# LIS-TU-Berlin/SVN-ICP

Measured on AMD Instinct MI355X. Metric: scan-pair registrations/sec at N particles x M source pts, 1/2/4/8 GPU, higher is better.
Workload: dtype f64; 1 GPU; C3: 128 particles SVN-ICP, 131072-pt source vs 262144-pt target, K=100, I=20, max_dist=1.0, lr=1.0, SVNFullGrad=False, correspondence=fast, early stop off; synthetic 64-beam scans (seed 20250718); particles=128, target_points=262144, knn_count=100, parallelism=single GPU

## Files before the change

### svn-icp_amd/csrc/api.hip

```cpp
#include "../../include/svnicp_hip.h"

#include <cmath>
#include <algorithm>
#include <cstdio>
#include <cstdlib>
#include <cstring>
#include <string>
#include <vector>

#include "device_buffer.hpp"
#include "kernels.hpp"
#include "stage_a_host.hpp"
#include "stage_b_host.hpp"

using namespace svnicp;
using namespace svnicp_host;

namespace {

struct CloudState {
  DevBuf<double> src, tgt;
  bool src_set = false, tgt_set = false;
};

// ... 313 lines not shown
  c->st.init_in_flight = true;
  c->st.host_stats_valid = false;
  const bool first = !c->run.particles_set || P != c->P;
  if (first && c->shard.row_world > 1) { c->shard.row_world = 1; c->shard.row_rank = 0; c->shard.B_total = 0; }
  c->P = P;
  if (!c->shard.set || first) { c->shard.p_lo = 0; c->shard.p_hi = P; c->shard.set = false; }
  HIPCHK(c, launch_init_particles(c->st.init_pose.p, P, c->pose0, c->prm.mode, c->st.R.p, c->st.t.p, c->st.Rtot.p, c->st.pose_out.p,
                                  (first || c->prm.mode == SVNICP_MODE_SVN) ? 1 : 0, c->st.eul.p, c->stream));
  c->run.particles_set = true;
  return SVNICP_OK;
}

int svnicp_set_initial_mean(svnicp_ctx* c, const double R0[9], const double t0[3]) {
  CTX_CHECK(c);
  if (!R0 || !t0) return fail(c, SVNICP_ERR_INVALID, "svnicp_set_initial_mean: null argument");
  std::memcpy(c->pose0.R0, R0, 9 * sizeof(double));
  std::memcpy(c->pose0.t0, t0, 3 * sizeof(double));
  c->run.have_candidates = false;
  return SVNICP_OK;
}

int svnicp_set_k(svnicp_ctx* c, int k) {
  CTX_CHECK(c);
  if (k < 1) return fail(c, SVNICP_ERR_INVALID, "svnicp_set_k: k >= 1 required");
  c->K = k;
  c->run.have_candidates = false;
  return SVNICP_OK;
}

int svnicp_set_max_dist(svnicp_ctx* c, double md) {
  CTX_CHECK(c);
  c->prm.max_dist = md;
  return SVNICP_OK;
}

int svnicp_set_option(svnicp_ctx* c, const char* name, const char* value) {
  CTX_CHECK(c);
  if (!name || !value) return fail(c, SVNICP_ERR_INVALID, "svnicp_set_option: null argument");
  const std::string k(name), v(value);
  Tuning& t = c->tune;
  auto num = [&](int lo, int hi, int* out) { char* end = nullptr; const long x = strtol(v.c_str(), &end, 10);
                                             if (end == v.c_str() || *end || x < lo || x > hi) return false; *out = (int)x; return true; };
  bool ok = true;
  if (k == "knn") { if (v == "auto") t.knn = {}; else if (v == "v1") t.knn = {false, KnnKernel::Stream}; else if (v == "v2") t.knn = {false, KnnKernel::SeededScan};
                    else if (v == "brute") t.knn = {false, KnnKernel::Brute}; else if (v == "tiles") t.knn = {false, KnnKernel::Tiles}; else ok = false; }
  else if (k == "fallback_sliced_max") ok = num(-1, 1 << 20, &t.fallback_sliced_max);
  else if (k == "accum") { if (v == "f64") t.accum = 0; else if (v == "valu") t.accum = 1; else if (v == "split") t.accum = 3; else ok = false; }
  else if (k == "update") { if (v == "auto") t.update_fused = 0; else if (v == "fused") t.update_fused = 1; else ok = false; }
  else if (k == "fused_update_max_p") ok = num(1, 700, &t.fused_update_max_p);
  else if (k == "wgpcu") { int x = 0, y = 0; ok = sscanf(v.c_str(), "%d,%d", &x, &y) == 2 && x >= 0 && x <= 64 && y >= 0 && y <= 16; if (ok) { t.wgpcu_search = x; t.wgpcu_accum = y; } }
  else if (k == "tp") ok = num(0, 1 << 16, &t.tp);
  else if (k == "debug") ok = num(0, 1, &t.debug);
  else if (k == "scan_split") ok = num(0, 16, &t.scan_split);
  else if (k == "group_stride") ok = num(0, 1 << 30, &t.group_stride);
  else if (k == "accum_min_steps") ok = num(0, 1 << 20, &t.accum_min_steps);
  else if (k == "brute_qb") { ok = num(0, 6, &t.brute_qb); }
  else if (k == "single") { if (v == "fused") t.single_fused = 1; else if (v == "split") t.single_fused = 0; else ok = false; }
  else if (k == "chain") { if (v == "auto") { t.small_chain = 1; t.persistent = 0; } else if (v == "persistent") { t.small_chain = 1; t.persistent = 1; }
                           else if (v == "general") { t.small_chain = 0; t.persistent = 0; } else ok = false; }
  else if (k == "median") { if (v == "auto") t.median_inline = -1; else if (v == "stream") t.median_inline = 0; else if (v == "inline") t.median_inline = 1; else ok = false; }
  else if (k == "correspondence") { if (v == "fast") t.full_corr = 0; else if (v == "full") t.full_corr = 1; else ok = false; }
  else return fail(c, SVNICP_ERR_INVALID, "svnicp_set_option: unknown option '" + k + "'");
  if (!ok) return fail(c, SVNICP_ERR_INVALID, "svnicp_set_option: bad value '" + v + "' for option '" + k + "'");
  c->run.have_candidates = false;
  c->sa.held = TargetLayout::None;
  if (c->run.began) c->st.step = plan_step(registration_facts(c, c->pl.on), c->tune, c->sb.plan);
  return SVNICP_OK;
}

int svnicp_set_shard(svnicp_ctx* c, int p_lo, int p_hi) {
  CTX_CHECK(c);
  if (!c->run.particles_set || p_lo < 0 || p_hi > c->P || p_lo > p_hi)
    return fail(c, SVNICP_ERR_INVALID, "svnicp_set_shard: need 0 <= p_lo <= p_hi <= P after svnicp_set_particles");
  c->shard.p_lo = p_lo; c->shard.p_hi = p_hi; c->shard.set = true;
  return SVNICP_OK;
}

int svnicp_set_row_shard(svnicp_ctx* c, int row_rank, int row_world, int64_t total_source_points) {
  CTX_CHECK(c);
  if (!c->run.particles_set || row_world < 1 || row_rank < 0 || row_rank >= row_world || (row_world > 1 && total_source_points < 1))
    return fail(c, SVNICP_ERR_INVALID, "svnicp_set_row_shard: need 0 <= row_rank < row_world and the whole scan's point count, after svnicp_set_particles");
  if (bind(c)) return SVNICP_ERR_HIP;
  c->shard.row_rank = row_rank; c->shard.row_world = row_world;
  c->shard.B_total = row_world > 1 ? total_source_points : 0;
  if (row_world > 1) {
    HIPCHK(c, c->shard.rank_sums.ensure((size_t)row_world * c->P * kNSums));
    HIPCHK(c, hipMemsetAsync(c->shard.rank_sums.p, 0, (size_t)row_world * c->P * kNSums * sizeof(double), c->stream));
  }
  return SVNICP_OK;
}

void* svnicp_rank_sums_devptr(svnicp_ctx* c) { return (c && c->shard.row_world > 1) ? (void*)c->shard.rank_sums.p : nullptr; }

static bool normal_pass_due(const svnicp_ctx* c) {
  return c->pl.on && !c->pl.supplied && !(c->pl.estimated && c->pl.est_k == c->pl.normal_k);
}

static int prepare_plane(svnicp_ctx* c);
int svnicp_align_begin(svnicp_ctx* c) {
  CTX_CHECK(c);
  if (!c->cloud.src_set || !c->cloud.tgt_set || !c->run.particles_set)
    return fail(c, SVNICP_ERR_INVALID, "svnicp_align: svnicp_set_clouds and svnicp_set_particles must come first");
  if (bind(c)) return SVNICP_ERR_HIP;
  const int I = c->prm.iterations, P = c->P;
  const int64_t B = c->B;
  const bool plane = c->pl.residual == SVNICP_RESIDUAL_PLANE;
// ... 774 lines not shown
```

### svn-icp_amd/csrc/kernels.hpp

```cpp
#pragma once
#include "device_math.hpp"
#include "registration_plan.hpp"
#include "stage_a_plan.hpp"

namespace svnicp {

struct KnnArgs {
  const double* src;
  Pose0 pose;
  const double *tx, *ty, *tz;
  const int32_t* torig;
  int64_t M, Mp;
  int64_t b_lo, b_hi;
  int K, S;
  double* pool_d;
  int32_t* pool_i;
  int32_t* out_idx;
  double* out_d2;
  const int32_t* qlist;
  const int* qlist_count;
  int list_grid;
  int list_qw;
  int slices, slice_max_queries, merge_n;
  double* sl_d;
// ... 7 lines not shown
  Pose0 pose;
  const double* tgt;
  int64_t M;
  int64_t b_lo, b_hi;
  int K;
  int32_t* out_idx;
  double* out_d2;
  unsigned long long* phase_cycles;
};
int knn_brute_queries_per_block(int64_t n, int num_cus);
hipError_t launch_knn_brute(const KnnBruteArgs& a, int num_cus, int queries_per_block, hipStream_t st);

struct KnnScanArgs {
  const double* src;
  Pose0 pose;
  const double *tx, *ty, *tz;
  const float *txf, *tyf, *tzf;
  const int32_t* torig;
  const unsigned long long* emax_bits;
  int64_t M, Mp, Ms;
  int64_t b_lo, b_hi;
  int K, S2, seed_rank;
  int32_t* pool;
  int32_t* out_idx;
  double* out_d2;
  int32_t* fail_list;
  int* fail_count;
};
hipError_t launch_targets_soa2(const double* tgt, int64_t M, int64_t Mp, double* tx, double* ty, double* tz,
                               float* txf, float* tyf, float* tzf, int32_t* torig, unsigned long long* emax_bits,
                               hipStream_t st);
hipError_t launch_knn_scan(const KnnScanArgs& a, hipStream_t st);
hipError_t launch_knn_topk(const KnnArgs& a, hipStream_t st);

struct KnnTilesArgs {
  const double* src;
  Pose0 pose;
  const int32_t* qorder;
  const double *tx, *ty, *tz;
  const float *txf, *tyf, *tzf;
  const int32_t* torig;
  const float* tile_box;
  const unsigned long long* emax_bits;
  int64_t M, Mp;
  int n_tiles;
  int64_t b_lo, b_hi;
  int K, S2;
  int32_t* pool;
  int32_t* arena;
  int32_t* chunk_tab;
  int arena_cap;
  int64_t tab_rows;
  int scan_split;
  unsigned int group_stride;
  int32_t* out_idx;
  double* out_d2;
  int32_t* fail_list;
  int* fail_count;
  int32_t* stat_n;
  unsigned long long* phase_cycles;
  void* qrec;
  double* fail_tau;
};
hipError_t launch_knn_tiles(const KnnTilesArgs& a, hipStream_t st);
size_t sort_temp_bytes(size_t n);
hipError_t launch_bbox(const double* pts, int64_t n, unsigned long long* bbox, hipStream_t st);
hipError_t launch_morton_order(const double* pts, int64_t i0, int64_t n, int transform, const Pose0& pose,
                               const unsigned long long* bbox, unsigned int* keys_a, unsigned int* keys_b,
                               int32_t* vals_a, int32_t* order, void* temp, size_t temp_bytes, hipStream_t st);
hipError_t launch_targets_sorted(const double* tgt, int64_t M, int64_t Mp, const int32_t* order, double* tx, double* ty,
                                 double* tz, float* txf, float* tyf, float* tzf, int32_t* torig, float* tile_box,
                                 unsigned long long* emax_bits, hipStream_t st);

struct AccumArgs {
  const double* src;
  const double* table;
  const float4* tablef;
  const float4* tablea;
  const float* cmax;
  int* ambig_count;
  const double* Rtot;
  int64_t B;
  int K, RS;
  int p_lo, p_hi;
  int TP;
  int tiles_per_block;
  int64_t n_tiles;
  int Ppad;
  double max_dist;
  double* partial;
  const int* ctl;
  int32_t* corr;
  int svgd;
  const double* tgt;
  const int32_t* cand;
  const double* anchor;
  int64_t M;
  uint8_t* kbest;
  int32_t* kidx;
  const int32_t* full_idx;
  int pts_per_block, spts_per_block;
  unsigned int* ticket;
  int fin_iteration, fin_P;
  double fin_thr;
  const double* fin_norms;
  const double* fin_pose;
// ... 121 lines not shown
```

### svn-icp_amd/csrc/knn_tiles.hip

```cpp
#include "kernels.hpp"

namespace svnicp {

namespace {

constexpr int T = 8;
constexpr int STEP = kWave * T;
constexpr int QW = 64;
constexpr int WAVES = 4;
constexpr int QCAP = 1024;
constexpr int SL = 512;
constexpr int NSQ = 4;
constexpr int MAX_TILES = 8192;
constexpr int QB = 16;
constexpr double kU = 5.9604644775390625e-08;

struct alignas(16) QF { float x, y, z, thr; };
struct alignas(16) QD { double x, y, z, tau; };

__device__ __forceinline__ void wave_sync() {
  __builtin_amdgcn_fence(__ATOMIC_ACQ_REL, "wavefront");
  __builtin_amdgcn_wave_barrier();
}
__device__ __forceinline__ bool ent_less(double da, int ia, double db, int ib) {
  return (da < db) || (da == db && ia < ib);
}
__device__ void bitonic_sort(double* sd, int* si, int S, int lane) {
  for (int k = 2; k <= S; k <<= 1)
    for (int j = k >> 1; j > 0; j >>= 1) {
      for (int e = lane; e < (S >> 1); e += kWave) {
        const int a = ((e & ~(j - 1)) << 1) | (e & (j - 1)), b = a | j;
        const bool up = (a & k) == 0;
        const double da = sd[a], db = sd[b];
        const int ia = si[a], ib = si[b];
        if (ent_less(db, ib, da, ia) == up) { sd[a] = db; si[a] = ib; sd[b] = da; si[b] = ia; }
      }
      wave_sync();
    }
}
__device__ void bitonic_sort128_f32(float* v, int lane) {
  for (int k = 2; k <= 128; k <<= 1)
    for (int j = k >> 1; j > 0; j >>= 1) {
      const int a = ((lane & ~(j - 1)) << 1) | (lane & (j - 1)), b = a | j;
      const bool up = (a & k) == 0;
      const float va = v[a], vb = v[b];
      if ((vb < va) == up) { v[a] = vb; v[b] = va; }
      wave_sync();
    }
}
__device__ __forceinline__ float next_down(float f) {
  if (f == 0.0f) return -1.401298464e-45f;
  int b = __float_as_int(f); b += (f > 0.0f) ? -1 : 1; return __int_as_float(b);
}
__device__ __forceinline__ float next_up(float f) {
  if (f == 0.0f) return 1.401298464e-45f;
  int b = __float_as_int(f); b += (f > 0.0f) ? 1 : -1; return __int_as_float(b);
}
__device__ __forceinline__ float f32_floor(double v) { float f = (float)v; return ((double)f > v) ? next_down(f) : f; }
__device__ __forceinline__ float f32_ceil(double v) { float f = (float)v; return ((double)f < v) ? next_up(f) : f; }
__device__ __forceinline__ float f32_round_up(double v) {
  float f = (float)v;
  if ((double)f < v) f = __int_as_float(__float_as_int(f) + 1);
  return f;
}
__device__ __forceinline__ float filter_threshold(double tau, double E) {
  if (!(tau < __builtin_huge_val())) return __builtin_huge_valf();
  const double r = sqrt(tau) * (1.0 + 1e-15) + 3.4641016151377553 * kU * E;
  return f32_round_up((r * r) * (1.0 + 5.0 * kU + 1e-6));
// ... 291 lines not shown
          for (int u = 0; u < NSQ; ++u) {
            const unsigned long long lo = key < best[u] ? key : best[u];
            key = key < best[u] ? best[u] : key;
            best[u] = lo;
          }
        }
        wave_sync();
      }
      if (lane < nq) {
#pragma unroll
        for (int i = 0; i < NSQ; ++i)
          if (best[i] != ~0ull) { const unsigned int t = (unsigned int)(best[i] & 0xffffffffull); atomicOr(&tbits[t >> 5], 1u << (t & 31)); }
      }
    }
    phase_mark(0);
    __syncthreads();
    phase_mark(3);
    const int qb0 = wave * QB;
    if (qb0 < nq) {
      const int nb = (nq - qb0) < QB ? (nq - qb0) : QB;
      for (int e = lane; e < QB * kWave; e += kWave) lm[e] = make_float2(__builtin_huge_valf(), __builtin_huge_valf());
      wave_sync();
      for (int wd = 0; wd < nwords; ++wd) {
        unsigned int bits = __builtin_amdgcn_readfirstlane(tbits[wd]);
        while (bits) {
          const int tile = (wd << 5) + (int)__builtin_ctz(bits);
          bits &= bits - 1;
          if (a.phase_cycles) pacc[4] += 1;
          const int64_t tb = (int64_t)tile * STEP;
          float x[T], y[T], z[T];
#pragma unroll
          for (int t = 0; t < T; ++t) { x[t] = a.txf[tb + t * kWave + lane]; y[t] = a.tyf[tb + t * kWave + lane]; z[t] = a.tzf[tb + t * kWave + lane]; }
          for (int q = 0; q < nb; ++q) {
            const float4 cur = *reinterpret_cast<const float4*>(&qf[qb0 + q]);
            float2 m = lm[q * kWave + lane];
#pragma unroll
            for (int t = 0; t < T; ++t) {
              const float dx = cur.x - x[t], dy = cur.y - y[t], dz = cur.z - z[t];
              float d = __builtin_fmaf(dz, dz, __builtin_fmaf(dy, dy, dx * dx));
              d = __builtin_fminf(d, __builtin_huge_valf());
              m.y = __builtin_amdgcn_fmed3f(m.x, m.y, d);
              m.x = __builtin_fminf(m.x, d);
            }
            lm[q * kWave + lane] = m;
          }
        }
      }
      wave_sync();
      phase_mark(5);
      for (int q = 0; q < nb; ++q) {
        const float2 m = lm[q * kWave + lane];
        const unsigned int kx = __float_as_uint(m.x), ky = __float_as_uint(m.y);
        unsigned int kth = 0u;
        for (int bit = 30; bit >= 0; --bit) {
          const unsigned int t_try = kth | ((1u << bit) - 1u);
          const int c = __popcll(__ballot(kx <= t_try)) + __popcll(__ballot(ky <= t_try));
          if (c < K) kth |= 1u << bit;
        }
        if (lane == 0) spare[qb0 + q] = (int)kth;
      }
      phase_mark(6);
    }
    phase_mark(1);
    __syncthreads();
    phase_mark(3);
    if (wave == 0 && lane < nq) {
      const double tv = (double)__uint_as_float((unsigned int)spare[lane]);
      const double E = fmax(Et, fmax(fabs(qd[lane].x), fmax(fabs(qd[lane].y), fabs(qd[lane].z))));
      double tau = __builtin_huge_val();
      if (tv < (double)__builtin_huge_valf()) {
        const double r = sqrt(tv) * (1.0 + 1e-6) + 4.0 * kU * E;
        tau = (r * r) * (1.0 + 1e-12);
      }
      qd[lane].tau = tau;
      const float thr = filter_threshold(tau, E);
      qf[lane].thr = thr;
      float tb = __builtin_huge_valf();
      if (thr < __builtin_huge_valf()) {
        const double rb = sqrt((double)thr) + 2.0 * kU * E;
        tb = f32_round_up((rb * rb) * (1.0 + 1e-6));
      }
      thrb[lane] = tb;
    }
    wave_sync();
  }

  if (wave == 0 && lane < nq) {
    QRec rec;
    rec.x = qd[lane].x; rec.y = qd[lane].y; rec.z = qd[lane].z; rec.tau = qd[lane].tau;
    rec.cnt = 0; rec.row = qb[lane]; rec.thr = qf[lane].thr; rec.tb = thrb[lane];
    reinterpret_cast<QRec*>(a.qrec)[q0 + lane] = rec;
  }
  phase_mark(1);
  if (a.phase_cycles && lane == 0) {
#pragma unroll
    for (int i = 0; i < 5; ++i) atomicAdd(&a.phase_cycles[i], pacc[i]);
    unsigned long long* pw = a.phase_cycles + 8 + 8 * ((size_t)grp * WAVES + wave);
#pragma unroll
    for (int i = 0; i < 7; ++i) pw[i] = pacc[i];
  }
}

template <int SW>
__global__ __launch_bounds__(64 * SW) void k_knn_scan_tiles(KnnTilesArgs a) {
  __shared__ __align__(16) QF s_qf[QW];
  __shared__ int s_cnt[QW];
  __shared__ int s_ticket;
  __shared__ __align__(16) int2 s_queue[SW][QCAP];
  const int lane = threadIdx.x & (kWave - 1);
  const int wave = __builtin_amdgcn_readfirstlane(threadIdx.x >> 6);
  const int S2 = a.S2, n_tiles = a.n_tiles;
  int2* queue = s_queue[wave];
  const unsigned int ngrp = gridDim.x;
  const unsigned int grp = (unsigned int)(((unsigned long long)blockIdx.x * a.group_stride) % ngrp);
  const int64_t q0 = a.b_lo + (int64_t)grp * QW;
  const int nq = (a.b_hi - q0) < QW ? (int)(a.b_hi - q0) : QW;
  QRec* recs = reinterpret_cast<QRec*>(a.qrec);
  unsigned long long tphase = a.phase_cycles ? __builtin_readcyclecounter() : 0ull;
  unsigned long long pacc[8] = {0, 0, 0, 0, 0, 0, 0, 0};
  auto phase_mark = [&](int i) {
    if (!a.phase_cycles) return;
    const unsigned long long now = __builtin_readcyclecounter();
    pacc[i] += now - tphase;
    tphase = now;
  };
  float gx = 0.f, gy = 0.f, gz = 0.f, gtb = -1.0f;
  float wlo0, wlo1, wlo2, whi0, whi1, whi2, tmax;
  {
    const bool act = lane < nq;
    QF f; f.x = f.y = f.z = 0.f; f.thr = -1.0f;
    const float inf = __builtin_huge_valf();
    wlo0 = wlo1 = wlo2 = inf; whi0 = whi1 = whi2 = -inf;
    if (act) {
      const QRec rec = recs[q0 + lane];
      f.x = (float)rec.x; f.y = (float)rec.y; f.z = (float)rec.z; f.thr = rec.thr;
      gtb = rec.tb;
      wlo0 = f32_floor(rec.x); wlo1 = f32_floor(rec.y); wlo2 = f32_floor(rec.z);
      whi0 = f32_ceil(rec.x); whi1 = f32_ceil(rec.y); whi2 = f32_ceil(rec.z);
    }
    gx = f.x; gy = f.y; gz = f.z;
    if (wave == 0) { s_qf[lane] = f; s_cnt[lane] = 0; }
    if (threadIdx.x == 0) s_ticket = 0;
    tmax = gtb;
    for (int off = 32; off > 0; off >>= 1) {
      wlo0 = __builtin_fminf(wlo0, __shfl_xor(wlo0, off, kWave)); whi0 = __builtin_fmaxf(whi0, __shfl_xor(whi0, off, kWave));
      wlo1 = __builtin_fminf(wlo1, __shfl_xor(wlo1, off, kWave)); whi1 = __builtin_fmaxf(whi1, __shfl_xor(whi1, off, kWave));
      wlo2 = __builtin_fminf(wlo2, __shfl_xor(wlo2, off, kWave)); whi2 = __builtin_fmaxf(whi2, __shfl_xor(whi2, off, kWave));
      tmax = __builtin_fmaxf(tmax, __shfl_xor(tmax, off, kWave));
    }
  }
  __syncthreads();
  const float* bx_lo0 = a.tile_box, *bx_lo1 = a.tile_box + n_tiles, *bx_lo2 = a.tile_box + 2 * (size_t)n_tiles;
  const float* bx_hi0 = a.tile_box + 3 * (size_t)n_tiles, *bx_hi1 = a.tile_box + 4 * (size_t)n_tiles,
             * bx_hi2 = a.tile_box + 5 * (size_t)n_tiles;
  int qcount = 0;
  auto put = [&](int q, int pos, bool on, int slot) {
    const int64_t r = q0 + q;
    if (on && pos < kTilesBase) a.pool[r * kTilesBase + pos] = slot;
    const bool ovf = on && pos >= kTilesBase && pos < S2;
    if (__ballot(ovf)) {
      const int o = pos - kTilesBase;
      int32_t* tab = a.chunk_tab + r * kTilesChunks + (ovf ? o / kTilesChunk : 0);
      if (ovf && (o % kTilesChunk) == 0) {
        int id = atomicAdd(a.chunk_tab + a.tab_rows * (int64_t)kTilesChunks, 1) + 1;
        if (id >= a.arena_cap) id = -2;
        __hip_atomic_store(tab, id, __ATOMIC_RELAXED, __HIP_MEMORY_SCOPE_AGENT);
      }
      if (ovf) {
        int id = -1;
        for (int spin = 0; spin < (1 << 22) && id == -1; ++spin) {
          id = __hip_atomic_load(tab, __ATOMIC_RELAXED, __HIP_MEMORY_SCOPE_AGENT);
          if (id == -1) __builtin_amdgcn_s_sleep(2);
        }
        if (id >= 0) a.arena[(int64_t)id * kTilesChunk + (o % kTilesChunk)] = slot;
        else atomicMax(&s_cnt[q], 1 << 24);
      }
    }
  };
  auto flush = [&]() {
    wave_sync();
    for (int e0 = 0; e0 < qcount; e0 += kWave) {
      const int e = e0 + lane;
      const bool on = e < qcount;
      const int2 ent = on ? queue[e] : make_int2(0, -1 - lane);
      const int prev = __shfl_up(ent.y, 1, kWave);
      const unsigned long long lead = __ballot(on && (lane == 0 || ent.y != prev));
      const unsigned long long upto = lead & (~0ull >> (63 - lane));
      const int L = 63 - (int)__builtin_clzll(upto | 1ull);
      const unsigned long long after = lead & ~((2ull << L) - 1ull);
      const int nvalid = (qcount - e0) < kWave ? (qcount - e0) : kWave;
      const int end = after ? (int)__builtin_ctzll(after) : nvalid;
      const int q = ent.y & (QW - 1);
      int base = 0;
      if (on && lane == L) base = atomicAdd(&s_cnt[q], end - L);
      base = __shfl(base, L, kWave);
      put(q, base + (lane - L), on, ent.x);
    }
    qcount = 0;
    wave_sync();
  };
  {
    auto next_ticket = [&]() { int v = 0; if (lane == 0) v = atomicAdd(&s_ticket, 1); return __builtin_amdgcn_readfirstlane(v); };
    int my = next_ticket(), seen = 0;
    for (int t0 = 0; t0 < n_tiles; t0 += kWave) {
      const int tl = t0 + lane;
      bool need = false;
      if (tl < n_tiles)
        need = box_lb2(wlo0, wlo1, wlo2, whi0, whi1, whi2, bx_lo0[tl], bx_lo1[tl], bx_lo2[tl], bx_hi0[tl], bx_hi1[tl], bx_hi2[tl]) <= tmax;
      const unsigned long long any = __ballot(need);
      const int n_here = __popcll(any);
      while (my < seen + n_here) {
        unsigned long long rem = any;
        for (int k = my - seen; k > 0; --k) rem &= rem - 1;
        const int tile = t0 + (int)__builtin_ctzll(rem);
        my = next_ticket();
        if (a.phase_cycles) pacc[5] += 1;
        const float l0 = bx_lo0[tile], l1 = bx_lo1[tile], l2 = bx_lo2[tile], h0 = bx_hi0[tile], h1 = bx_hi1[tile], h2 = bx_hi2[tile];
        unsigned long long qmask = __ballot(lane < nq && box_lb2(gx, gy, gz, gx, gy, gz, l0, l1, l2, h0, h1, h2) <= gtb);
        if (!qmask) continue;
        if (a.phase_cycles) pacc[6] += __popcll(qmask);
        const int64_t tb = (int64_t)tile * STEP;
        float x[T], y[T], z[T];
#pragma unroll
        for (int t = 0; t < T; ++t) { x[t] = a.txf[tb + t * kWave + lane]; y[t] = a.tyf[tb + t * kWave + lane]; z[t] = a.tzf[tb + t * kWave + lane]; }
        while (qmask) {
          const int q = (int)__builtin_ctzll(qmask);
          qmask &= qmask - 1;
          const float4 cur = *reinterpret_cast<const float4*>(&s_qf[q]);
          float d[T];
#pragma unroll
          for (int t = 0; t < T; ++t) {
            const float dx = cur.x - x[t], dy = cur.y - y[t], dz = cur.z - z[t];
            d[t] = __builtin_fmaf(dz, dz, __builtin_fmaf(dy, dy, dx * dx));
          }
          float dm = __builtin_fminf(__builtin_fminf(d[0], d[1]), d[2]);
#pragma unroll
          for (int t = 3; t + 1 < T; t += 2) dm = __builtin_fminf(__builtin_fminf(dm, d[t]), d[t + 1]);
          if constexpr ((T - 3) % 2 == 1) dm = __builtin_fminf(dm, d[T - 1]);
          if (__ballot(dm <= cur.w)) {
#pragma unroll
            for (int t = 0; t < T; ++t) {
              const bool hit = d[t] <= cur.w;
              const unsigned long long m = __ballot(hit);
              if (m) {
                const int pos = qcount + (int)__builtin_amdgcn_mbcnt_hi((unsigned int)(m >> 32), __builtin_amdgcn_mbcnt_lo((unsigned int)m, 0u));
                if (hit) queue[pos] = make_int2((int)(tb + t * kWave + lane), q);
                qcount += __popcll(m);
              }
            }
            qcount = __builtin_amdgcn_readfirstlane(qcount);
            if (qcount > QCAP - STEP) flush();
          }
        }
      }
      seen += n_here;
    }
    flush();
  }
  phase_mark(2);
  __syncthreads();
  phase_mark(3);
  if (wave == 0 && lane < nq) recs[q0 + lane].cnt = s_cnt[lane];
  if (a.phase_cycles && lane == 0) {
    atomicAdd(&a.phase_cycles[2], pacc[2]); atomicAdd(&a.phase_cycles[3], pacc[3]);
    atomicAdd(&a.phase_cycles[5], pacc[5]); atomicAdd(&a.phase_cycles[6], pacc[6]);
    atomicMax(&a.phase_cycles[7], pacc[2]);
  }
}

__global__ __launch_bounds__(256) void k_knn_select(KnnTilesArgs a) {
  __shared__ __align__(16) double s_sd[WAVES][SL];
  __shared__ int s_si[WAVES][SL];
  const int lane = threadIdx.x & (kWave - 1);
  const int wave = __builtin_amdgcn_readfirstlane(threadIdx.x >> 6);
  const QRec* recs = reinterpret_cast<const QRec*>(a.qrec);
  for (int64_t r = a.b_lo + (int64_t)blockIdx.x * WAVES + wave; r < a.b_hi; r += (int64_t)gridDim.x * WAVES) {
    const QRec rec = recs[r];
    select_query(a, r, rec, s_sd[wave], s_si[wave], lane);
  }
}

}

static_assert(STEP == kTileSlots && MAX_TILES == kMaxTiles, "knn_tiles_applicable (stage_a_plan.hpp) speaks of this kernel's tiles");

hipError_t launch_knn_tiles(const KnnTilesArgs& a, hipStream_t st) {
  const int64_t nq = a.b_hi - a.b_lo;
  if (nq <= 0) return hipSuccess;
  const int64_t nb = (nq + QW - 1) / QW;
  if (a.n_tiles > MAX_TILES) return hipErrorInvalidValue;
  const size_t smem = sizeof(QD) * QW + sizeof(QF) * QW + 4 * sizeof(int) * QW + sizeof(unsigned int) * (MAX_TILES / 32) +
                      (sizeof(float2) * QB * kWave + 512) * WAVES;
  hipError_t e = hipFuncSetAttribute(reinterpret_cast<const void*>(k_knn_seed),
                                     hipFuncAttributeMaxDynamicSharedMemorySize, (int)smem);
  if (e != hipSuccess) return e;
  hipLaunchKernelGGL(k_knn_seed, dim3((unsigned)nb), dim3(256), smem, st, a);
  e = hipGetLastError();
  if (e != hipSuccess) return e;
  if (a.scan_split == 4) hipLaunchKernelGGL(k_knn_scan_tiles<4>, dim3((unsigned)((nq + QW - 1) / QW)), dim3(256), 0, st, a);
  else hipLaunchKernelGGL(k_knn_scan_tiles<8>, dim3((unsigned)((nq + QW - 1) / QW)), dim3(512), 0, st, a);
  e = hipGetLastError();
  if (e != hipSuccess) return e;
  int64_t nbs = (nq + WAVES - 1) / WAVES;
  if (nbs > 65536) nbs = 65536;
  hipLaunchKernelGGL(k_knn_select, dim3((unsigned)nbs), dim3(256), 0, st, a);
  return hipGetLastError();
}

}
```

### svn-icp_amd/csrc/registration_plan.hpp

```cpp
#pragma once
#include <cstddef>
#include <cstdint>
#include <initializer_list>

#include "stage_a_plan.hpp"

namespace svnicp {

struct Tuning {
  KnnOption knn;
  int fallback_sliced_max = -1;
  int accum = 3;
  int update_fused = 0;
  int fused_update_max_p = 128;
  int wgpcu_search = 0, wgpcu_accum = 0;
  int tp = 0;
  int accum_min_steps = 0;
  int group_stride = 0;
  int scan_split = 0;
  int debug = 0;
  int single_fused = 1;
  int small_chain = 1;
  int persistent = 0;
  int median_inline = -1;
  int brute_qb = 0;
  int full_corr = 0;
};

struct RegistrationFacts {
  int P = 0, K = 0, I = 0;
  int64_t B = 0, M = 0;
  bool svgd = false, check_early_stop = false, record_trace = false;
  bool profiling = false;
  bool shard_set = false;
  int p_lo = 0, p_hi = 0;
  int row_world = 1;
  int batch = 0;
  bool explicit_tab = false;
  int tab_I = 0;
  bool plane = false;
  bool normals_supplied = false;
  int normal_k = 16;
  int nshard() const { return p_hi - p_lo; }
  bool whole_shard() const { return p_lo == 0 && p_hi == P; }
};

constexpr int64_t kMinibatchMaxRows = 1ll << 22;
struct RegistrationRows {
  bool mb;
  int64_t Bq;
  int64_t Bt;
  int64_t Bi;
};
inline RegistrationRows registration_rows(int batch, int I, int64_t B) {
  if (batch == 0 || I <= 0) return {false, B, B, B};
  const int64_t n = (int64_t)I * batch;
  return {true, B < n ? B : n, n, batch};
}

struct Refusal { bool holds; const char* why; };
inline const char* first_refusal(std::initializer_list<Refusal> ladder) {
  for (const Refusal& r : ladder)
    if (r.holds) return r.why;
  return nullptr;
}
constexpr const char* kMinibatchRefusal = "svnicp_align: mini-batch mode (svnicp_set_minibatch) is not available here: ";
constexpr const char* kPlaneRefusal = "svnicp_align: the point-to-plane residual (svnicp_set_residual) is not available here: ";

inline const char* minibatch_refusal(const RegistrationFacts& f, const Tuning& t) {
  if (f.batch == 0) return nullptr;
  return first_refusal({
      {f.batch < 0, "batch_size must be positive"},
// ... 107 lines not shown
```

### svn-icp_amd/csrc/stage_a_host.hpp

```cpp
#pragma once
#include <algorithm>
#include <cstdio>
#include <initializer_list>
#include <vector>

#include "device_buffer.hpp"
#include "kernels.hpp"

namespace svnicp_host {
using namespace svnicp;

struct StageAEnv {
  hipStream_t stream;
  const Tuning& tune;
  int num_cus;
  bool record_trace;
  const double* tgt;
  int64_t B, M;
  const Pose0& pose0;
};

struct StageA {
  StageAPlan plan;
  TargetLayout held = TargetLayout::None;
// ... 54 lines not shown
    HIPCHK(o, torig.ensure(Mp)); HIPCHK(o, emax.ensure(1));
    if (plan.layout == TargetLayout::Morton) {
      const size_t nmax = std::max(M, B);
      HIPCHK(o, keys_a.ensure(nmax)); HIPCHK(o, keys_b.ensure(nmax)); HIPCHK(o, vals_a.ensure(nmax));
      HIPCHK(o, order_t.ensure(M)); HIPCHK(o, qorder.ensure(B));
      HIPCHK(o, bbox.ensure(6)); HIPCHK(o, tile_box.ensure(6 * (Mp / kTileSlots)));
      if (nmax > sort_n) { sort_tmp_bytes = sort_temp_bytes(nmax); HIPCHK(o, sort_tmp.ensure(sort_tmp_bytes)); sort_n = nmax; }
    }
    if (held == plan.layout) return SVNICP_OK;
    if (plan.layout == TargetLayout::Hashed) {
      HIPCHK(o, launch_targets_soa2(e.tgt, e.M, plan.Mp, tx.p, ty.p, tz.p, txf.p, tyf.p, tzf.p, torig.p, emax.p, e.stream));
    } else {
      HIPCHK(o, launch_bbox(e.tgt, e.M, bbox.p, e.stream));
      HIPCHK(o, launch_morton_order(e.tgt, 0, e.M, 0, e.pose0, bbox.p, keys_a.p, keys_b.p, vals_a.p, order_t.p, sort_tmp.p, sort_tmp_bytes, e.stream));
      HIPCHK(o, launch_targets_sorted(e.tgt, e.M, plan.Mp, order_t.p, tx.p, ty.p, tz.p, txf.p, tyf.p, tzf.p, torig.p, tile_box.p, emax.p, e.stream));
    }
    held = plan.layout;
    return SVNICP_OK;
  }

  hipError_t launch_fallback(KnnArgs a, hipStream_t stream) {
    a.qlist = fail_list.p; a.qlist_count = fail_count.p; a.list_grid = kFallbackGrid; a.list_qw = kFallbackQW;
    a.slice_max_queries = plan.sliced_max; a.slices = 0;
    hipError_t e = launch_knn_topk(a, stream);
    if (e != hipSuccess || plan.sliced_max <= 0) return e;
    a.slices = knn_slice_count(a.K);
    a.merge_n = 1;
    while (a.merge_n < a.slices * a.K) a.merge_n <<= 1;
    a.sl_d = sl_d.p; a.sl_i = sl_i.p;
    e = launch_knn_topk(a, stream);
    if (e != hipSuccess) return e;
    return launch_knn_merge_slices(a, stream);
  }

  template <class Obj>
  int clear_dbg_phase(Obj* o, hipStream_t stream, size_t waves) {
    HIPCHK(o, dbg_phase.ensure(8 + 8 * kDbgPhaseWaves));
    HIPCHK(o, hipMemsetAsync(dbg_phase.p, 0, (8 + 8 * waves) * sizeof(unsigned long long), stream));
    return SVNICP_OK;
  }

  template <class Obj>
  int print_phases(Obj* o, const StageAEnv& e, int64_t n, size_t dbg_waves) {
    std::vector<unsigned long long> h(8 + 8 * dbg_waves);
    HIPCHK(o, hipMemcpyAsync(h.data(), dbg_phase.p, h.size() * sizeof(unsigned long long), hipMemcpyDeviceToHost, e.stream));
    HIPCHK(o, hipStreamSynchronize(e.stream));
    if (plan.kernel == KnnKernel::Brute) {
      const int qb = e.tune.brute_qb > 0 ? e.tune.brute_qb : knn_brute_queries_per_block(n, e.num_cus);
      const double nwg = (double)((n + qb - 1) / qb);
      fprintf(stderr, "[svnicp] k_knn_brute (%d queries per workgroup) thread-0 cycles per workgroup: pass A %.0f, bound %.0f, pass B %.0f, general path %.0f, rank + write %.0f\n",
              qb, h[0] / nwg, h[1] / nwg, h[2] / nwg, h[3] / nwg, h[4] / nwg);
      return SVNICP_OK;
    }
    fprintf(stderr, "[svnicp] k_knn_tiles wave cycles: rank %llu seed %llu scan %llu barrier waits + hand-over %llu | counts: seed tiles %llu scan tiles %llu scan (query, tile) pairs %llu\n", h[0], h[1], h[2], h[3], h[4], h[5], h[6]);
    auto column = [&](const char* tag, int col, unsigned long long floor_) {
      std::vector<unsigned long long> v;
      for (size_t w = 0; w < dbg_waves; ++w) { const unsigned long long x = h[8 + 8 * w + col]; if (x >= floor_) v.push_back(x); }
      if (v.empty()) return;
      std::sort(v.begin(), v.end());
      fprintf(stderr, "[svnicp]   seed kernel %-12s n %6zu  p50 %8llu  p90 %8llu  p99 %8llu  max %8llu cycles\n", tag, v.size(), v[v.size() / 2],
              v[v.size() * 9 / 10], v[v.size() * 99 / 100], v.back());
    };
    column("rank", 0, 5000); column("seed", 1, 1); column("tile loop", 5, 1); column("bisection", 6, 1); column("waits", 3, 0);
    return SVNICP_OK;
  }

  template <class Obj>
  int search(Obj* o, const StageAEnv& e, const double* qsrc, const Pose0& pose, int K, int32_t* out_idx, double* out_d2, int64_t b_lo,
             int64_t b_hi) {
    const int64_t n = b_hi - b_lo;
    KnnArgs a{};
    a.src = qsrc; a.pose = pose; a.tx = tx.p; a.ty = ty.p; a.tz = tz.p; a.torig = torig.p;
    a.M = e.M; a.Mp = plan.Mp; a.b_lo = b_lo; a.b_hi = b_hi; a.K = K; a.S = knn_pool_size(K);
    a.pool_d = pool_d.p; a.pool_i = pool_i.p; a.out_idx = out_idx; a.out_d2 = out_d2;
    switch (plan.kernel) {
    case KnnKernel::Brute: {
      KnnBruteArgs k{};
      k.src = qsrc; k.pose = pose; k.tgt = e.tgt; k.M = e.M; k.b_lo = b_lo; k.b_hi = b_hi; k.K = K; k.out_idx = out_idx; k.out_d2 = out_d2;
      if (e.tune.debug) {
        if (const int rc = clear_dbg_phase(o, e.stream, 0)) return rc;
        k.phase_cycles = dbg_phase.p;
      }
      HIPCHK(o, launch_knn_brute(k, e.num_cus, e.tune.brute_qb, e.stream));
      if (e.tune.debug) return print_phases(o, e, n, 0);
      return SVNICP_OK;
    }
    case KnnKernel::Tiles: {
      if (n <= 0) return SVNICP_OK;
      HIPCHK(o, launch_morton_order(qsrc, b_lo, n, 1, pose, bbox.p, keys_a.p, keys_b.p, vals_a.p, qorder.p + b_lo, sort_tmp.p, sort_tmp_bytes, e.stream));
      KnnTilesArgs k{};
      k.src = qsrc; k.pose = pose; k.qorder = qorder.p + b_lo;
      k.tx = tx.p; k.ty = ty.p; k.tz = tz.p; k.txf = txf.p; k.tyf = tyf.p; k.tzf = tzf.p;
      k.torig = torig.p; k.tile_box = tile_box.p; k.emax_bits = emax.p;
      k.M = e.M; k.Mp = plan.Mp; k.n_tiles = (int)(plan.Mp / kTileSlots); k.b_lo = b_lo; k.b_hi = b_hi; k.K = K; k.S2 = plan.S2;
      k.pool = pool2.p; k.out_idx = out_idx; k.out_d2 = out_d2;
      k.arena = arena.p; k.chunk_tab = chunk_tab.p; k.arena_cap = plan.arena_cap; k.tab_rows = plan.rows;
      k.scan_split = e.tune.scan_split == 4 ? 4 : 8;
      {
        const unsigned int ng = (unsigned int)((n + 63) / 64);
        unsigned int st = e.tune.group_stride > 0 ? (unsigned int)e.tune.group_stride : 17u;
        auto gcd = [](unsigned int x, unsigned int y) { while (y) { const unsigned int t = x % y; x = y; y = t; } return x; };
        while (st > 1 && gcd(st, ng) != 1) st += 2;
        if (ng <= 2 || st >= ng) st = 1;
        k.group_stride = st;
      }
      HIPCHK(o, hipMemsetAsync(chunk_tab.p, 0xff, tiles_chunk_tab_words(plan.rows) * sizeof(int32_t), e.stream));
      k.fail_list = fail_list.p; k.fail_count = fail_count.p; k.fail_tau = fail_tau.p; k.qrec = qrec.p;
      a.qthr = fail_tau.p;
      if (e.record_trace) k.stat_n = stat_n.p;
      HIPCHK(o, hipMemsetAsync(fail_count.p, 0, sizeof(int), e.stream));
      const size_t dbg_waves = (size_t)((n + 63) / 64) * 4;
      const bool dbg = e.tune.debug && dbg_waves <= kDbgPhaseWaves;
      if (dbg) {
        if (const int rc = clear_dbg_phase(o, e.stream, dbg_waves)) return rc;
        k.phase_cycles = dbg_phase.p;
      }
      HIPCHK(o, launch_knn_tiles(k, e.stream));
      if (dbg)
        if (const int rc = print_phases(o, e, n, dbg_waves)) return rc;
      HIPCHK(o, launch_fallback(a, e.stream));
      return SVNICP_OK;
    }
    case KnnKernel::SeededScan: {
      KnnScanArgs k{};
      k.src = qsrc; k.pose = pose; k.tx = tx.p; k.ty = ty.p; k.tz = tz.p;
      k.txf = txf.p; k.tyf = tyf.p; k.tzf = tzf.p; k.torig = torig.p; k.emax_bits = emax.p;
      k.M = e.M; k.Mp = plan.Mp; k.Ms = plan.scan_Ms; k.b_lo = b_lo; k.b_hi = b_hi; k.K = K; k.S2 = plan.S2;
      k.seed_rank = plan.scan_rank; k.pool = pool2.p; k.out_idx = out_idx; k.out_d2 = out_d2;
      k.fail_list = fail_list.p; k.fail_count = fail_count.p;
      HIPCHK(o, hipMemsetAsync(fail_count.p, 0, sizeof(int), e.stream));
      HIPCHK(o, launch_knn_scan(k, e.stream));
      HIPCHK(o, launch_fallback(a, e.stream));
      return SVNICP_OK;
    }
    case KnnKernel::Stream:
      HIPCHK(o, launch_knn_topk(a, e.stream));
    }
    return SVNICP_OK;
  }

  int64_t block_rows(int64_t n) const { return std::max<int64_t>(1, std::min<int64_t>(plan.rows, n)); }
  template <class Obj, class Done = int (*)(int64_t, int64_t)>
  int search_blocks(Obj* o, const StageAEnv& e, const double* q, int64_t n, int Kq, int32_t* out_idx, double* out_d2, int out_step,
                    Done done = [](int64_t, int64_t) { return 0; }) {
    Pose0 ident{};
    ident.R0[0] = ident.R0[4] = ident.R0[8] = 1.0;
    const int64_t rows = block_rows(n);
    for (int64_t lo = 0; lo < n; lo += rows) {
      const int64_t cnt = std::min<int64_t>(rows, n - lo), off = lo * out_step * Kq;
      if (const int rc = search(o, e, q + 3 * lo, ident, Kq, out_idx + off, out_d2 + off, 0, cnt)) return rc;
// ... 24 lines not shown
```

### svn-icp_amd/csrc/stage_a_plan.hpp

```cpp
#pragma once
#include <cstddef>
#include <cstdint>

namespace svnicp {

enum class KnnKernel { Stream , SeededScan , Tiles , Brute  };
struct KnnOption { bool automatic = true; KnnKernel kernel = KnnKernel::Stream; };
enum class TargetLayout { None, Hashed, Morton };

constexpr int kTileSlots = 512;
constexpr int kMaxTiles = 8192;
constexpr int kTilesBase = 512, kTilesChunk = 512, kTilesChunks = 31;
constexpr int kMatrixKMax = 128;
constexpr int kScanKMax = 200;
constexpr double kBrutePairsMax = 268435456.0;
constexpr int kFallbackGrid = 256;
constexpr int kFallbackSlicedMax = 512;
constexpr int kFallbackQW = 2;

inline int64_t knn_padded_targets(int64_t M) { return ((M + kTileSlots - 1) / kTileSlots) * kTileSlots; }
inline int knn_pool_size(int K) {
  int S = 256;
  while (S < K + 128) S <<= 1;
  return S;
}
inline int knn_slice_count(int K) {
  int kp = 1;
  while (kp < K) kp <<= 1;
  int ns = 8192 / kp;
  return ns > 64 ? 64 : (ns < 1 ? 1 : ns);
}
inline bool knn_tiles_applicable(int64_t Mp, int K) {
  return K <= kMatrixKMax && Mp >= 16 * kTileSlots && (Mp % kTileSlots) == 0 && Mp / kTileSlots <= kMaxTiles;
}
inline bool knn_scan_plan(int64_t Mp, int K, int64_t* Ms, int* seed_rank, int* S2) {
  if (K > kScanKMax || Mp < 16 * kTileSlots || (Mp % kTileSlots) != 0) return false;
  double F = 12.5 / (double)K;
  if (F > 0.25) F = 0.25;
  int64_t ms = (int64_t)((double)Mp * F / kTileSlots + 0.5) * kTileSlots;
  if (ms < kTileSlots) ms = kTileSlots;
  if (ms > Mp) ms = Mp;
  int j = (int)(2.6 * (double)K * (double)ms / (double)Mp + 0.5);
  if (j < 4) j = 4;
  if (j > 44) j = 44;
  *Ms = ms;
  *seed_rank = j - 1;
  *S2 = 1024;
  return true;
}
inline bool knn_brute_applicable(int64_t B, int64_t M, int K) {
  return K >= 1 && K <= kMatrixKMax && B >= 1 && M >= 1 && M < (1ll << 31) && (double)B * (double)M <= kBrutePairsMax;
}
inline size_t tiles_chunk_tab_words(int64_t rows) { return (size_t)rows * kTilesChunks + 16 + (size_t)(rows + 63) / 64 + 1; }

struct StageAPlan {
  KnnKernel kernel = KnnKernel::Stream;
  TargetLayout layout = TargetLayout::Hashed;
  int64_t rows = 0, Mp = 0;
  int K = 0;
  int64_t scan_Ms = 0;
  int scan_rank = 0;
  int S2 = 0;
  int sliced_max = 0;
  int arena_cap = 0;
  bool has_fallback() const { return kernel == KnnKernel::SeededScan || kernel == KnnKernel::Tiles; }
  bool can_search(int Kq) const {
    if (kernel == KnnKernel::SeededScan) return Kq == K;
    return kernel == KnnKernel::Stream || Kq <= kMatrixKMax;
  }
};

inline StageAPlan plan_stage_a(int64_t rows, int64_t M, int K, KnnOption opt, int fallback_sliced_max) {
  StageAPlan p;
  p.rows = rows; p.K = K; p.Mp = knn_padded_targets(M);
  const bool scan_ok = knn_scan_plan(p.Mp, K, &p.scan_Ms, &p.scan_rank, &p.S2);
  p.kernel = knn_tiles_applicable(p.Mp, K) ? KnnKernel::Tiles : scan_ok ? KnnKernel::SeededScan : KnnKernel::Stream;
  if (opt.automatic) {
    if (knn_brute_applicable(rows, M, K)) p.kernel = KnnKernel::Brute;
  } else if (opt.kernel == KnnKernel::Stream) {
    p.kernel = KnnKernel::Stream;
  } else if (opt.kernel == KnnKernel::SeededScan) {
    p.kernel = scan_ok ? KnnKernel::SeededScan : KnnKernel::Stream;
  } else if (opt.kernel == KnnKernel::Brute && K <= kMatrixKMax && M < (1ll << 31)) {
    p.kernel = KnnKernel::Brute;
  }
  p.layout = p.kernel == KnnKernel::Brute ? TargetLayout::None : p.kernel == KnnKernel::Tiles ? TargetLayout::Morton : TargetLayout::Hashed;
  if (p.kernel == KnnKernel::Tiles) {
    p.S2 = kTilesBase + kTilesChunks * kTilesChunk;
    p.arena_cap = (int)(rows / 4 > 32768 ? rows / 4 : 32768);
  }
  if (p.has_fallback()) {
    p.sliced_max = fallback_sliced_max >= 0 && fallback_sliced_max < kFallbackSlicedMax ? fallback_sliced_max : kFallbackSlicedMax;
  }
  return p;
}

}
```

Baseline: 145.3 registrations/s.

## Split tile scan work into query sub-blocks and truncate seed bisection bits

Tile-scan work units in the tiles KNN kernel become (tile, query sub-block) pairs, so a tile's matching queries can be spread over up to four waves. This is meant to balance the per-tile scan work across more waves when targets are few relative to queries. A host heuristic picks 1/2/4 units from the query-to-target ratio. The seed kth-distance bisection also stops after 5 mantissa bits and rounds the threshold up, giving a looser but cheaper seed bound. The cost is more ticket traffic, repeated box tests, and more candidate work from the looser threshold.

```diff
diff --git a/svn-icp_amd/csrc/api.hip b/svn-icp_amd/csrc/api.hip
--- a/svn-icp_amd/csrc/api.hip
+++ b/svn-icp_amd/csrc/api.hip
@@ -389,6 +389,7 @@
   else if (k == "tp") ok = num(0, 1 << 16, &t.tp);
   else if (k == "debug") ok = num(0, 1, &t.debug);
   else if (k == "scan_split") ok = num(0, 16, &t.scan_split);
+  else if (k == "scan_units") { int u = 0; ok = num(0, 4, &u) && u != 3; if (ok) t.scan_units = u; }
   else if (k == "group_stride") ok = num(0, 1 << 30, &t.group_stride);
   else if (k == "accum_min_steps") ok = num(0, 1 << 20, &t.accum_min_steps);
   else if (k == "brute_qb") { ok = num(0, 6, &t.brute_qb); }
diff --git a/svn-icp_amd/csrc/kernels.hpp b/svn-icp_amd/csrc/kernels.hpp
--- a/svn-icp_amd/csrc/kernels.hpp
+++ b/svn-icp_amd/csrc/kernels.hpp
@@ -83,6 +83,7 @@
   int arena_cap;
   int64_t tab_rows;
   int scan_split;
+  int scan_units;
   unsigned int group_stride;
   int32_t* out_idx;
   double* out_d2;
diff --git a/svn-icp_amd/csrc/knn_tiles.hip b/svn-icp_amd/csrc/knn_tiles.hip
--- a/svn-icp_amd/csrc/knn_tiles.hip
+++ b/svn-icp_amd/csrc/knn_tiles.hip
@@ -14,6 +14,8 @@
 constexpr int MAX_TILES = 8192;
 constexpr int QB = 16;
 constexpr double kU = 5.9604644775390625e-08;
+constexpr int kSeedMantBits = 5;
+static_assert(kSeedMantBits >= 0 && kSeedMantBits <= 23, "float32 has 23 mantissa bits");
 
 struct alignas(16) QF { float x, y, z, thr; };
 struct alignas(16) QD { double x, y, z, tau; };
@@ -411,11 +413,12 @@
         const float2 m = lm[q * kWave + lane];
         const unsigned int kx = __float_as_uint(m.x), ky = __float_as_uint(m.y);
         unsigned int kth = 0u;
-        for (int bit = 30; bit >= 0; --bit) {
+        for (int bit = 30; bit >= 23 - kSeedMantBits; --bit) {
           const unsigned int t_try = kth | ((1u << bit) - 1u);
           const int c = __popcll(__ballot(kx <= t_try)) + __popcll(__ballot(ky <= t_try));
           if (c < K) kth |= 1u << bit;
         }
+        kth |= (1u << (23 - kSeedMantBits)) - 1u;
         if (lane == 0) spare[qb0 + q] = (int)kth;
       }
       phase_mark(6);
@@ -460,8 +463,9 @@
   }
 }
 
-template <int SW>
+template <int SW, int NQ>
 __global__ __launch_bounds__(64 * SW) void k_knn_scan_tiles(KnnTilesArgs a) {
+  static_assert(NQ == 1 || NQ == 2 || NQ == 4, "a query block is 64 / NQ consecutive lanes");
   __shared__ __align__(16) QF s_qf[QW];
   __shared__ int s_cnt[QW];
   __shared__ int s_ticket;
@@ -560,6 +564,7 @@
   };
   {
     auto next_ticket = [&]() { int v = 0; if (lane == 0) v = atomicAdd(&s_ticket, 1); return __builtin_amdgcn_readfirstlane(v); };
+    constexpr int QBLK = QW / NQ;
     int my = next_ticket(), seen = 0;
     for (int t0 = 0; t0 < n_tiles; t0 += kWave) {
       const int tl = t0 + lane;
@@ -568,14 +573,16 @@
         need = box_lb2(wlo0, wlo1, wlo2, whi0, whi1, whi2, bx_lo0[tl], bx_lo1[tl], bx_lo2[tl], bx_hi0[tl], bx_hi1[tl], bx_hi2[tl]) <= tmax;
       const unsigned long long any = __ballot(need);
       const int n_here = __popcll(any);
-      while (my < seen + n_here) {
+      while (my / NQ < seen + n_here) {
         unsigned long long rem = any;
-        for (int k = my - seen; k > 0; --k) rem &= rem - 1;
+        for (int k = my / NQ - seen; k > 0; --k) rem &= rem - 1;
         const int tile = t0 + (int)__builtin_ctzll(rem);
+        const int blk = my % NQ;
         my = next_ticket();
         if (a.phase_cycles) pacc[5] += 1;
         const float l0 = bx_lo0[tile], l1 = bx_lo1[tile], l2 = bx_lo2[tile], h0 = bx_hi0[tile], h1 = bx_hi1[tile], h2 = bx_hi2[tile];
         unsigned long long qmask = __ballot(lane < nq && box_lb2(gx, gy, gz, gx, gy, gz, l0, l1, l2, h0, h1, h2) <= gtb);
+        if constexpr (NQ > 1) qmask &= (~0ull >> (QW - QBLK)) << (blk * QBLK);
         if (!qmask) continue;
         if (a.phase_cycles) pacc[6] += __popcll(qmask);
         const int64_t tb = (int64_t)tile * STEP;
@@ -648,6 +655,8 @@
   if (nq <= 0) return hipSuccess;
   const int64_t nb = (nq + QW - 1) / QW;
   if (a.n_tiles > MAX_TILES) return hipErrorInvalidValue;
+  const int units = a.scan_units;
+  if (units != 1 && units != 2 && units != 4) return hipErrorInvalidValue;
   const size_t smem = sizeof(QD) * QW + sizeof(QF) * QW + 4 * sizeof(int) * QW + sizeof(unsigned int) * (MAX_TILES / 32) +
                       (sizeof(float2) * QB * kWave + 512) * WAVES;
   hipError_t e = hipFuncSetAttribute(reinterpret_cast<const void*>(k_knn_seed),
@@ -656,8 +665,11 @@
   hipLaunchKernelGGL(k_knn_seed, dim3((unsigned)nb), dim3(256), smem, st, a);
   e = hipGetLastError();
   if (e != hipSuccess) return e;
-  if (a.scan_split == 4) hipLaunchKernelGGL(k_knn_scan_tiles<4>, dim3((unsigned)((nq + QW - 1) / QW)), dim3(256), 0, st, a);
-  else hipLaunchKernelGGL(k_knn_scan_tiles<8>, dim3((unsigned)((nq + QW - 1) / QW)), dim3(512), 0, st, a);
+  const dim3 sgrid((unsigned)((nq + QW - 1) / QW));
+#define SVNICP_SCAN(SW, NQ) hipLaunchKernelGGL((k_knn_scan_tiles<SW, NQ>), sgrid, dim3(64 * SW), 0, st, a)
+  if (a.scan_split == 4) { if (units == 1) SVNICP_SCAN(4, 1); else if (units == 2) SVNICP_SCAN(4, 2); else SVNICP_SCAN(4, 4); }
+  else { if (units == 1) SVNICP_SCAN(8, 1); else if (units == 2) SVNICP_SCAN(8, 2); else SVNICP_SCAN(8, 4); }
+#undef SVNICP_SCAN
   e = hipGetLastError();
   if (e != hipSuccess) return e;
   int64_t nbs = (nq + WAVES - 1) / WAVES;
diff --git a/svn-icp_amd/csrc/registration_plan.hpp b/svn-icp_amd/csrc/registration_plan.hpp
--- a/svn-icp_amd/csrc/registration_plan.hpp
+++ b/svn-icp_amd/csrc/registration_plan.hpp
@@ -18,6 +18,7 @@
   int accum_min_steps = 0;
   int group_stride = 0;
   int scan_split = 0;
+  int scan_units = 0;
   int debug = 0;
   int single_fused = 1;
   int small_chain = 1;
diff --git a/svn-icp_amd/csrc/stage_a_host.hpp b/svn-icp_amd/csrc/stage_a_host.hpp
--- a/svn-icp_amd/csrc/stage_a_host.hpp
+++ b/svn-icp_amd/csrc/stage_a_host.hpp
@@ -130,7 +130,7 @@
               qb, h[0] / nwg, h[1] / nwg, h[2] / nwg, h[3] / nwg, h[4] / nwg);
       return SVNICP_OK;
     }
-    fprintf(stderr, "[svnicp] k_knn_tiles wave cycles: rank %llu seed %llu scan %llu barrier waits + hand-over %llu | counts: seed tiles %llu scan tiles %llu scan (query, tile) pairs %llu\n", h[0], h[1], h[2], h[3], h[4], h[5], h[6]);
+    fprintf(stderr, "[svnicp] k_knn_tiles wave cycles: rank %llu seed %llu scan %llu barrier waits + hand-over %llu | counts: seed tiles %llu scan units (tile, query block) %llu scan (query, tile) pairs %llu\n", h[0], h[1], h[2], h[3], h[4], h[5], h[6]);
     auto column = [&](const char* tag, int col, unsigned long long floor_) {
       std::vector<unsigned long long> v;
       for (size_t w = 0; w < dbg_waves; ++w) { const unsigned long long x = h[8 + 8 * w + col]; if (x >= floor_) v.push_back(x); }
@@ -139,6 +139,11 @@
       fprintf(stderr, "[svnicp]   seed kernel %-12s n %6zu  p50 %8llu  p90 %8llu  p99 %8llu  max %8llu cycles\n", tag, v.size(), v[v.size() / 2],
               v[v.size() * 9 / 10], v[v.size() * 99 / 100], v.back());
     };
+    unsigned long long seed_waits = 0;
+    for (size_t w = 0; w < dbg_waves; ++w) seed_waits += h[8 + 8 * w + 3];
+    const unsigned long long scan_waits = h[3] - seed_waits;
+    fprintf(stderr, "[svnicp]   scan kernel wave cycles: tile loop %llu, final barrier %llu (%.1f %% of both), slowest wave's tile loop %llu\n", h[2], scan_waits,
+            100.0 * (double)scan_waits / (double)(h[2] + scan_waits + 1), h[7]);
     column("rank", 0, 5000); column("seed", 1, 1); column("tile loop", 5, 1); column("bisection", 6, 1); column("waits", 3, 0);
     return SVNICP_OK;
   }
@@ -174,6 +179,7 @@
       k.pool = pool2.p; k.out_idx = out_idx; k.out_d2 = out_d2;
       k.arena = arena.p; k.chunk_tab = chunk_tab.p; k.arena_cap = plan.arena_cap; k.tab_rows = plan.rows;
       k.scan_split = e.tune.scan_split == 4 ? 4 : 8;
+      k.scan_units = knn_scan_units(n, e.M, e.tune.scan_units);
       {
         const unsigned int ng = (unsigned int)((n + 63) / 64);
         unsigned int st = e.tune.group_stride > 0 ? (unsigned int)e.tune.group_stride : 17u;
diff --git a/svn-icp_amd/csrc/stage_a_plan.hpp b/svn-icp_amd/csrc/stage_a_plan.hpp
--- a/svn-icp_amd/csrc/stage_a_plan.hpp
+++ b/svn-icp_amd/csrc/stage_a_plan.hpp
@@ -51,6 +51,10 @@
 inline bool knn_brute_applicable(int64_t B, int64_t M, int K) {
   return K >= 1 && K <= kMatrixKMax && B >= 1 && M >= 1 && M < (1ll << 31) && (double)B * (double)M <= kBrutePairsMax;
 }
+inline int knn_scan_units(int64_t queries, int64_t M, int option) {
+  if (option == 1 || option == 2 || option == 4) return option;
+  return M <= 2 * queries ? 4 : M <= 4 * queries ? 2 : 1;
+}
 inline size_t tiles_chunk_tab_words(int64_t rows) { return (size_t)rows * kTilesChunks + 16 + (size_t)(rows + 63) / 64 + 1; }
 
 struct StageAPlan {
```

Result: faster. 148.0 registrations/s, median of 6 (+1.9%).
